# d-f/nylon-amt

Measured on AMD Instinct MI355X. Metric: training clips/sec (128-frame x 256-bin), higher is better.
Workload: dtype f16x3 (split fp16 / bf16 operand pairs, three bf16-rate MFMA passes per product, fp32 accumulate; tensors that flow between kernels are fp32 (attention q/k/v as fp16 hi+lo pairs), the copies SAVED only for the backward -- FFN hidden, its gradient, pre-LayerNorm sums -- are bf16); 1 GPU; paper-size hFT-Transformer training step (d=256, ff=512, 3+3 layers, 4 heads), batch 8 clips/GPU, dropout 0.10, forward+loss+backward+Adam; global_batch=8, frames=128, bins=256, parallelism=dp1, precision_mode=x3

## Files before the change

### nylon-amt_amd/csrc/x3_strip.hip

```cpp
#include <stdlib.h>
#include <type_traits>
#include <utility>
#include "hftt_common.h"
#include "x3_common.h"
#include "hftt_launch.h"
#include "x3_internal.h"
#include "../../include/hftt_hip.h"

#ifdef HFTT_X3_STRIP_ABLATE
#define XDBG(g, bit) (((g).pad & (bit)) != 0)
#else
#define XDBG(g, bit) false
#endif

namespace {

#include "strip_pipe.h"

__host__ __device__ inline int x3_i_of_c(int c) { const int g = c & 15, hh = c >> 4; return (g & 3) + 8 * (g >> 2) + 4 * hh; }

template <int E>
__global__ __launch_bounds__(256) void x3_strip_pack_kernel(const float* __restrict__ params, unsigned short* __restrict__ dst,
                                                            const hftt_strip_pack_entry* __restrict__ table) {
  const hftt_strip_pack_entry e = table[blockIdx.y];
  const int nrows = e.transpose ? e.cols : e.rows;
  const int nk = e.transpose ? e.rows : e.cols;
  const int kch = nk >> 3;
  const long total = (long)nrows * kch;
  for (long t = (long)blockIdx.x * 256 + threadIdx.x; t < total; t += (long)gridDim.x * 256) {
    const int nl = (int)(t / kch), kc = (int)(t - (long)nl * kch);
    const int n = e.n0 + nl, k = e.k0 + kc * 8;
    float v[8];
    const float* src = params + e.src_off;
    if (e.transpose) {
#pragma unroll
      for (int q = 0; q < 8; q++) v[q] = src[(long)(kc * 8 + q) * e.src_ld + nl];
    } else {
      const float4 a = *reinterpret_cast<const float4*>(src + (long)nl * e.src_ld + kc * 8);
      const float4 b = *reinterpret_cast<const float4*>(src + (long)nl * e.src_ld + kc * 8 + 4);
      v[0] = a.x; v[1] = a.y; v[2] = a.z; v[3] = a.w; v[4] = b.x; v[5] = b.y; v[6] = b.z; v[7] = b.w;
    }
    const int tile = n >> 5, i = x3_i_of_c(n & 31);
    const int pt = k >> 5, hk2 = (k >> 4) & 1, u = (k >> 3) & 1;
    const int ch = 2 * pt + u;
    long off;
    if (e.order == 2) {
      off = (e.slot_offset + (long)ch * e.slot_stride + tile) * 1024 + (hk2 * 32 + i) * 8;
    } else {
      long slot, frag;
      if (e.order == 0) { slot = (long)(tile >> 3) * (e.K >> 4) + ch; frag = 2 * (tile & 7); }
      else { slot = 2 * tile + (ch >> 3); frag = 2 * (ch & 7); }
      const long pos = e.slot_offset + (long)e.slot_stride * (slot >> 1) + (slot & 1);
      off = (pos * 16 + frag) * 512 + (hk2 * 32 + i) * 8;
    }
    bf16x8 hi, lo;
    x3_split8_checked<E>(v, hi, lo);
    *reinterpret_cast<bf16x8*>(dst + e.dst_off + off) = hi;
    *reinterpret_cast<bf16x8*>(dst + e.dst_off + off + 512) = lo;
  }
}

struct XPipe {
  const unsigned short* w;
  int S;
  int fill_pos;
  unsigned ring;
  int wave, lane;
  bool nofill, nobar;
  __device__ __forceinline__ const unsigned short* src_of(int pos) const { return w + ((long)pos * 16 + wave * 4) * 512 + lane * 8; }
  __device__ __forceinline__ void advance() { fill_pos = (fill_pos + 1 == S) ? 0 : fill_pos + 1; }
  template <int BUF>
  __device__ __forceinline__ void fill() {
    glds16x4(src_of(fill_pos), ring + (unsigned)BUF * SLOT_BYTES + (unsigned)wave * 4096u);
    advance();
  }
  __device__ __forceinline__ void begin_slot() {
    if (!nobar) { HFTT_WAITVM(4); __builtin_amdgcn_s_barrier(); }
  }
  __device__ __forceinline__ void prologue_sync() { HFTT_WAITVM(4); __builtin_amdgcn_s_barrier(); }
  template <int BUF>
  __device__ __forceinline__ void refill() {
    if (!nofill) glds16x4(src_of(fill_pos), ring + (unsigned)((BUF + FILL_AHEAD) & (NSLOT - 1)) * SLOT_BYTES + (unsigned)wave * 4096u);
    advance();
  }
  __device__ __forceinline__ void drain() { HFTT_WAITVM(0); }
};

struct XChunk { u4v a, b; };
#ifndef HFTT_STRIP_NT
#define HFTT_STRIP_NT 2
#endif
__device__ __forceinline__ u4v stream_load16(const void* p) {
#if HFTT_STRIP_NT == 1
  return __builtin_nontemporal_load(reinterpret_cast<const u4v*>(p));
#else
  return *reinterpret_cast<const u4v*>(p);
#endif
}
__device__ __forceinline__ void stream_store16(void* p, const u4v& v) {
#if HFTT_STRIP_NT
  __builtin_nontemporal_store(v, reinterpret_cast<u4v*>(p));
#else
  *reinterpret_cast<u4v*>(p) = v;
#endif
}
__device__ __forceinline__ void chunk_load(XChunk& c, const float* p) {
  c.a = stream_load16(p);
  c.b = stream_load16(p + 4);
}
template <typename V>
__device__ __forceinline__ void chunk_raw(XChunk& c, const V& v, int at = 0) {
  c.a = u4v{__float_as_uint(v[at]), __float_as_uint(v[at + 1]), __float_as_uint(v[at + 2]), __float_as_uint(v[at + 3])};
  c.b = u4v{__float_as_uint(v[at + 4]), __float_as_uint(v[at + 5]), __float_as_uint(v[at + 6]), __float_as_uint(v[at + 7])};
}
__device__ __forceinline__ void chunk_floats(const XChunk& c, float* v) {
  v[0] = __uint_as_float(c.a.x); v[1] = __uint_as_float(c.a.y); v[2] = __uint_as_float(c.a.z); v[3] = __uint_as_float(c.a.w);
  v[4] = __uint_as_float(c.b.x); v[5] = __uint_as_float(c.b.y); v[6] = __uint_as_float(c.b.z); v[7] = __uint_as_float(c.b.w);
}
template <int E>
__device__ __forceinline__ void x3_split16(const float* v, XChunk (&hf)[2]) {
#pragma unroll
  for (int u = 0; u < 2; u++) {
    bf16x8 hi, lo;
    x3_split8<E>(v + 8 * u, hi, lo);
    hf[u].a = __builtin_bit_cast(u4v, hi); hf[u].b = __builtin_bit_cast(u4v, lo);
  }
}
template <int E>
__device__ __forceinline__ void chunk_convert(XChunk& c) {
  float v[8];
  chunk_floats(c, v);
  bf16x8 hi, lo;
  if (E == X3_BF16H) {
    uint4 h;
    h.x = X3<E>::pk(v[0], v[1]); h.y = X3<E>::pk(v[2], v[3]); h.z = X3<E>::pk(v[4], v[5]); h.w = X3<E>::pk(v[6], v[7]);
    c.a = __builtin_bit_cast(u4v, h);
    return;
  }
  x3_split8<E>(v, hi, lo);
  c.a = __builtin_bit_cast(u4v, hi); c.b = __builtin_bit_cast(u4v, lo);
}
__device__ __forceinline__ void chunk_drop(XChunk& c, uint64_t seed, uint32_t site, uint64_t q0, uint32_t thr, float inv_keep) {
  float v[8];
  chunk_floats(c, v);
  drop8(v, seed, site, q0, thr, inv_keep);
  chunk_raw(c, v);
}
template <int E>
__device__ __forceinline__ void chunk_values(const XChunk& c, float* v) {
  const unsigned h[4] = {c.a.x, c.a.y, c.a.z, c.a.w}, l[4] = {c.b.x, c.b.y, c.b.z, c.b.w};
#pragma unroll
  for (int q = 0; q < 4; q++) {
    float h0, h1, l0, l1;
    X3<E>::unpk(h[q], h0, h1); X3<E>::unpk(l[q], l0, l1);
    v[2 * q] = h0 + l0; v[2 * q + 1] = h1 + l1;
  }
}
__device__ __forceinline__ int chunk_off(int ch) { return (ch >> 1) * 32 + (ch & 1) * 8; }

struct XPre { bf16x8 f[4]; bool noread = false; };
__device__ __forceinline__ void slot_head(const unsigned char* slot, XPre& pre) {
#pragma unroll
  for (int i = 0; i < 4; i++) pre.f[i] = *reinterpret_cast<const bf16x8*>(slot + i * 1024);
}
template <int E, typename G>
__device__ __forceinline__ void x3_slot_tiles(const unsigned char* slot, const unsigned char* next, XPre& pre, const XChunk& x, f32x16 (&acc)[8], G&& side) {
  bf16x8 fr[16];
#pragma unroll
  for (int i = 0; i < 4; i++) fr[i] = pre.f[i];
  const bf16x8 xh = __builtin_bit_cast(bf16x8, x.a), xl = __builtin_bit_cast(bf16x8, x.b);
  static_for<8>([&](auto t_c) __attribute__((always_inline)) {
    constexpr int t = decltype(t_c)::value;
    acc[t] = X3<E>::mma(fr[2 * t + 1], xh, acc[t]);
    side(std::integral_constant<int, 3 * t>{});
    if (pre.noread) { if (2 * t + 4 < 16) fr[2 * t + 4] = fr[2 * t]; }
    else if (2 * t + 4 < 16) fr[2 * t + 4] = *reinterpret_cast<const bf16x8*>(slot + (2 * t + 4) * 1024);
    else pre.f[2 * t + 4 - 16] = *reinterpret_cast<const bf16x8*>(next + (2 * t + 4 - 16) * 1024);
    if (E != X3_BF16H) acc[t] = X3<E>::mma(fr[2 * t], xl, acc[t]);
    side(std::integral_constant<int, 3 * t + 1>{});
    if (pre.noread) { if (2 * t + 5 < 16) fr[2 * t + 5] = fr[2 * t + 1]; }
    else if (2 * t + 5 < 16) fr[2 * t + 5] = *reinterpret_cast<const bf16x8*>(slot + (2 * t + 5) * 1024);
    else pre.f[2 * t + 5 - 16] = *reinterpret_cast<const bf16x8*>(next + (2 * t + 5 - 16) * 1024);
    acc[t] = X3<E>::mma(fr[2 * t], xh, acc[t]);
    side(std::integral_constant<int, 3 * t + 2>{});
    __builtin_amdgcn_sched_barrier(0);
  });
}
template <int E, int OFF, typename G>
__device__ __forceinline__ void x3_slot_chunks(const unsigned char* slot, const unsigned char* next, XPre& pre, const XChunk (&x)[16], f32x16& acc, G&& side) {
  bf16x8 fr[16];
#pragma unroll
  for (int i = 0; i < 4; i++) fr[i] = pre.f[i];
  static_for<8>([&](auto q_c) __attribute__((always_inline)) {
    constexpr int q = decltype(q_c)::value;
    const bf16x8 xh = __builtin_bit_cast(bf16x8, x[OFF + q].a), xl = __builtin_bit_cast(bf16x8, x[OFF + q].b);
    acc = X3<E>::mma(fr[2 * q + 1], xh, acc);
    side(std::integral_constant<int, 3 * q>{});
    if (pre.noread) { if (2 * q + 4 < 16) fr[2 * q + 4] = fr[2 * q]; }
    else if (2 * q + 4 < 16) fr[2 * q + 4] = *reinterpret_cast<const bf16x8*>(slot + (2 * q + 4) * 1024);
    else pre.f[2 * q + 4 - 16] = *reinterpret_cast<const bf16x8*>(next + (2 * q + 4 - 16) * 1024);
    if (E != X3_BF16H) acc = X3<E>::mma(fr[2 * q], xl, acc);
    side(std::integral_constant<int, 3 * q + 1>{});
    if (pre.noread) { if (2 * q + 5 < 16) fr[2 * q + 5] = fr[2 * q + 1]; }
    else if (2 * q + 5 < 16) fr[2 * q + 5] = *reinterpret_cast<const bf16x8*>(slot + (2 * q + 5) * 1024);
    else pre.f[2 * q + 5 - 16] = *reinterpret_cast<const bf16x8*>(next + (2 * q + 5 - 16) * 1024);
    acc = X3<E>::mma(fr[2 * q], xh, acc);
    side(std::integral_constant<int, 3 * q + 2>{});
    __builtin_amdgcn_sched_barrier(0);
  });
}

__device__ __forceinline__ f32x16 acc_from_lds(const float* row) {
  float b[16];
  lds16f(row, b);
  f32x16 acc;
#pragma unroll
  for (int q = 0; q < 16; q++) acc[q] = b[q];
  return acc;
}
__device__ __forceinline__ void acc_from_lds(f32x16 (&acc)[8], const float* row) {
#pragma unroll
  for (int ot = 0; ot < 8; ot++) acc[ot] = acc_from_lds(row + ot * 32);
}

__device__ __forceinline__ void load16f(const float* p, float* v) {
#pragma unroll
  for (int q = 0; q < 4; q++) { const float4 t = reinterpret_cast<const float4*>(p)[q]; v[4 * q] = t.x; v[4 * q + 1] = t.y; v[4 * q + 2] = t.z; v[4 * q + 3] = t.w; }
}
__device__ __forceinline__ void store16f(float* p, const float* v) {
#pragma unroll
// ... 231 lines not shown
          tile_store_rows(stage, v, j, hb, lane, cwave + ot * 32, g.ldc, wave_ok && !dbg_nostore);
        }
        __builtin_amdgcn_sched_barrier(0);
      }
      if (LN) {
        const bool p16 = g.flags & HFTT_SL_PRE_BF16;
        x3_ln_rows(acc, prm_b + g.N, prm_b + g.N + 256, hb, g.ln_mean, g.ln_rstd, tok, wave_ok, stage, j, lane,
                   (preb != nullptr && !p16) ? preb + (blk * 128 + wave * 32) * g.ldc : nullptr, cwave, g.ldc,
                   (preb != nullptr && p16) ? reinterpret_cast<unsigned short*>(preb) + (blk * 128 + wave * 32) * g.ldc : nullptr);
      }
    }
  }
  P.drain();
}

template <int E, int NT, bool HR, bool PLN = false, bool XD = false>
__global__ __launch_bounds__(256, 2) void x3_linear_n_kernel(const hftt_strip_desc g) {
  static_assert(!PLN || (E == X3_F16 && !HR), "f16-pair output: a forward projection without residual");
  static_assert(!XD || (E != X3_F16 && !PLN), "masked strip: a backward product");
  extern __shared__ __attribute__((aligned(16))) unsigned char smem[];
  const int tid = threadIdx.x, lane = tid & 63;
  const int wave = __builtin_amdgcn_readfirstlane(tid >> 6);
  const int j = lane & 31, h = lane >> 5;
  const long nblk = ((long)g.M + 127) / 128;
  float* prm = reinterpret_cast<float*>(smem + RING_BYTES);
  float* stage = reinterpret_cast<float*>(smem + RING_BYTES + 4 * NT * 32 + wave * STG_BYTES_PER_WAVE);
  const float* xb = reinterpret_cast<const float*>(g.x);
  float* cb = reinterpret_cast<float*>(g.C);
  const float* rb = reinterpret_cast<const float*>(g.residual);
  const bool relu = g.flags & HFTT_SL_RELU;
  const bool dbg_nostore = XDBG(g, 16);

  auto tok_of = [&](long blk) { const long t = blk * 128 + wave * 32 + j; return t < g.M ? t : (long)g.M - 1; };
  for (int i = tid; i < g.N; i += 256) prm[i] = g.bias != nullptr ? g.bias[i] : 0.f;
  XChunk xr[16];
  XPipe P = x3_open(g.w, 2 * NT, smem, wave, lane, XDBG(g, 1), XDBG(g, 2), xr, xb + tok_of(blockIdx.x) * g.ldx + 16 * h);

  const uint32_t thr = hftt_keep_thr(g.drop_p);
  const float inv_keep = hftt_keep_scale(g.drop_p);
  const unsigned char* abase = smem + lane * 16;
  for (long blk = blockIdx.x; blk < nblk; blk += gridDim.x) {
    int hb = h;
    asm volatile("" : "+v"(hb));
    const bool wave_ok = (blk * 128 + wave * 32) < g.M;
    const long nxt = blk + gridDim.x;
    auto lane_tok = [&](long b) { int l_ = lane; asm volatile("" : "+v"(l_)); const long t = b * 128 + wave * 32 + (l_ & 31); return t < g.M ? t : (long)g.M - 1; };
    float* cwave = cb + (blk * 128 + wave * 32) * g.ldc;
    int zero = 0;
    asm volatile("" : "+s"(zero));
    const float* prm_b = prm + zero;
    if (XD && g.drop_p > 0.f) {
      const uint64_t rowq_x = ((uint64_t)lane_tok(blk) * (uint64_t)g.K) >> 2;
#pragma unroll
      for (int c = 0; c < 16; c++) chunk_drop(xr[c], g.drop_seed, g.drop_site, rowq_x + ((chunk_off(c) + 16 * hb) >> 2), thr, inv_keep);
    }
#pragma unroll
    for (int c = 0; c < 16; c++) chunk_convert<E>(xr[c]);
    XPre pre;
    slot_head(abase, pre);

    for (int tp = 0; tp < NT / 2; tp++)
    static_for<2>([&](auto hf_c) __attribute__((always_inline)) {
      constexpr int half = decltype(hf_c)::value;
      constexpr int BA = (2 * half) & 3, BB = (2 * half + 1) & 3;
      const int t = 2 * tp + half;
      const bool LAST = (t == NT - 1);
      f32x16 hacc;
      {
        float b[16];
        lds16f(prm_b + t * 32 + 16 * hb, b);
#pragma unroll
        for (int q = 0; q < 16; q++) hacc[q] = b[q];
      }
      float r[16];
      P.begin_slot();
      x3_slot_chunks<E, 0>(abase + BA * SLOT_BYTES, abase + BB * SLOT_BYTES, pre, xr, hacc, [&](auto i_c) __attribute__((always_inline)) {
        constexpr int i = decltype(i_c)::value;
        if (i == 1) P.template refill<BA>();
        if (i == 4 && HR) {
          const long tokc = lane_tok(blk);
          const long rrow = g.res_mod > 0 ? (long)((unsigned)tokc % (unsigned)g.res_mod) : tokc;
          load16f(rb + rrow * g.ldr + 16 * hb + t * 32, r);
        }
        if (LAST && i % 3 == 2) chunk_load(xr[i / 3], xb + lane_tok(nxt < nblk ? nxt : blk) * g.ldx + 16 * hb + chunk_off(i / 3));
      });
      P.begin_slot();
      x3_slot_chunks<E, 8>(abase + BB * SLOT_BYTES, abase + ((BB + 1) & 3) * SLOT_BYTES, pre, xr, hacc, [&](auto i_c) __attribute__((always_inline)) {
        constexpr int i = decltype(i_c)::value;
        if (i == 1) P.template refill<BB>();
        if (LAST && i % 3 == 2) chunk_load(xr[8 + i / 3], xb + lane_tok(nxt < nblk ? nxt : blk) * g.ldx + 16 * hb + chunk_off(8 + i / 3));
      });
      float v[16];
#pragma unroll
      for (int q = 0; q < 16; q++) {
        float a = hacc[q];
        if (relu) a = fmaxf(a, 0.f);
        v[q] = a * g.out_scale;
      }
      if (!XD && g.drop_p > 0.f) {
        int l_ = lane; asm volatile("" : "+v"(l_));
        const uint64_t rowq = ((uint64_t)(blk * 128 + wave * 32 + (l_ & 31)) * (uint64_t)g.N) >> 2;
        drop16(v, g.drop_seed, g.drop_site, rowq + ((t * 32 + 16 * hb) >> 2), thr, inv_keep);
      }
      if (HR) {
#pragma unroll
        for (int q = 0; q < 16; q++) v[q] += r[q];
      }
      if (PLN) tile_store_rows_f16pair(stage, v, j, hb, lane, cwave + t * 32, g.ldc, wave_ok && !dbg_nostore);
      else tile_store_rows(stage, v, j, hb, lane, cwave + t * 32, g.ldc, wave_ok && !dbg_nostore);
    });
  }
  P.drain();
}

struct XNoHead {};
template <int MODE, int PT, bool HH, bool GH, bool HEAD, typename O>
__device__ __forceinline__ void x3_mlp_block(const O& o, const hftt_ffn_desc& g) {
  static_assert(!HEAD || MODE == 0, "the fc_o head belongs to the forward block");
  constexpr int E = (MODE == 0) ? X3_F16 : (GH ? X3_BF16H : X3_BF16);
  extern __shared__ __attribute__((aligned(16))) unsigned char smem[];
  const int tid = threadIdx.x, lane = tid & 63;
  const int wave = __builtin_amdgcn_readfirstlane(tid >> 6);
  const int j = lane & 31, h = lane >> 5;
  constexpr int p = PT * 32;
  constexpr int HP = HEAD ? 768 : 0;
  const long nblk = ((long)g.M + 127) / 128;
  float* prm_head = reinterpret_cast<float*>(smem + RING_BYTES);
  float* prm = prm_head + HP;
  float* stage = reinterpret_cast<float*>(smem + RING_BYTES + 4 * (HP + PT * 32 + 768) + wave * STG_BYTES_PER_WAVE);
  const float* xb;
  long ldx;
  if constexpr (HEAD) { xb = reinterpret_cast<const float*>(o.x); ldx = o.ldx; }
  else { xb = reinterpret_cast<const float*>(g.x); ldx = g.ldx; }
  float* yb = reinterpret_cast<float*>(g.y);
  float* preb = reinterpret_cast<float*>(g.pre_ln_out);
  const float* rb = reinterpret_cast<const float*>(g.residual);
  float* hob = reinterpret_cast<float*>(g.h_out);
  const float* gtb = reinterpret_cast<const float*>(g.gate);
  unsigned short* hob16 = reinterpret_cast<unsigned short*>(g.h_out);
  const unsigned short* gtb16 = reinterpret_cast<const unsigned short*>(g.gate);
  const bool has_res = (MODE == 1) && g.residual != nullptr;

  auto tok_of = [&](long blk) { const long t = blk * 128 + wave * 32 + j; return t < g.M ? t : (long)g.M - 1; };

  if constexpr (HEAD) {
    prm_head[tid] = o.bias != nullptr ? o.bias[tid] : 0.f;
    prm_head[256 + tid] = o.ln_gamma[tid]; prm_head[512 + tid] = o.ln_beta[tid];
  }
  for (int i = tid; i < p; i += 256) prm[i] = (MODE == 0 && g.b1 != nullptr) ? g.b1[i] : 0.f;
  prm[p + tid] = (MODE == 0 && g.b2 != nullptr) ? g.b2[tid] : 0.f;
  if (MODE == 0) { prm[p + 256 + tid] = g.ln_gamma[tid]; prm[p + 512 + tid] = g.ln_beta[tid]; }

  XChunk xr[16];
  const unsigned short* wstream;
  if constexpr (HEAD) wstream = o.w; else wstream = g.w;
  XPipe P = x3_open(wstream, (HEAD ? 16 : 0) + 4 * PT, smem, wave, lane, XDBG(g, 1), XDBG(g, 2), xr, xb + tok_of(blockIdx.x) * ldx + 16 * h);

  const uint32_t thr = hftt_keep_thr(g.drop_p);
  const float inv_keep = hftt_keep_scale(g.drop_p);
  uint32_t thr_a = 0;
  float inv_keep_a = 1.f;
  if constexpr (HEAD) { thr_a = hftt_keep_thr(o.drop_p); inv_keep_a = hftt_keep_scale(o.drop_p); }
  const unsigned char* abase = smem + lane * 16;
  for (long blk = blockIdx.x; blk < nblk; blk += gridDim.x) {
    int hb = h;
    asm volatile("" : "+v"(hb));
    const long tok = blk * 128 + wave * 32 + j;
    const bool wave_ok = (blk * 128 + wave * 32) < g.M;
    const long tokc = tok_of(blk);
    const long nxt = blk + gridDim.x;
    int zero = 0;
    asm volatile("" : "+s"(zero));
    const float* prm_b = prm + zero;
    const float* xrow_next = xb + (nxt < nblk ? tok_of(nxt) : tokc) * ldx + 16 * hb;
    const uint64_t rowq_h = ((uint64_t)tok * (uint64_t)p) >> 2;

    if constexpr (HEAD) {
      const float* prm_a = prm_b - HP;
      chunk_convert<E>(xr[0]);
      f32x16 acc[8];
      acc_from_lds(acc, prm_a + 16 * hb);
      XPre pre;
      slot_head(abase, pre);
      x3_kouter_slots<E>(P, abase, pre, xr, acc, false, true, nullptr, nullptr);
      const uint64_t rowq_a = ((uint64_t)tok * 256ull) >> 2;
      const long rrow = o.res_mod > 0 ? (long)((unsigned)tokc % (unsigned)o.res_mod) : tokc;
      const float* rrow_p = reinterpret_cast<const float*>(o.residual) + rrow * o.ldr + 16 * hb;
      float rnext[16];
      load16f(rrow_p, rnext);
#pragma unroll
      for (int ot = 0; ot < 8; ot++) {
        const int col0 = ot * 32 + 16 * hb;
        float v[16], r[16];
#pragma unroll
        for (int q = 0; q < 16; q++) r[q] = rnext[q];
        if (ot < 7) load16f(rrow_p + (ot + 1) * 32, rnext);
#pragma unroll
        for (int q = 0; q < 16; q++) v[q] = acc[ot][q] * o.out_scale;
        if (o.drop_p > 0.f) drop16(v, o.drop_seed, o.drop_site, rowq_a + (col0 >> 2), thr_a, inv_keep_a);
#pragma unroll
        for (int q = 0; q < 16; q++) acc[ot][q] = v[q] + r[q];
        __builtin_amdgcn_sched_barrier(0);
      }
      float* pre1b = reinterpret_cast<float*>(o.pre_ln_out);
      float* y1b = reinterpret_cast<float*>(o.C);
      const bool p16a = o.flags & HFTT_SL_PRE_BF16;
      x3_ln_rows<true>(acc, prm_a + 256, prm_a + 512, hb, o.ln_mean, o.ln_rstd, tok, wave_ok, stage, j, lane,
                       (pre1b != nullptr && !p16a) ? pre1b + (blk * 128 + wave * 32) * o.ldc : nullptr,
                       y1b != nullptr ? y1b + (blk * 128 + wave * 32) * o.ldc : nullptr, o.ldc,
                       (pre1b != nullptr && p16a) ? reinterpret_cast<unsigned short*>(pre1b) + (blk * 128 + wave * 32) * o.ldc : nullptr);
#pragma unroll
      for (int c = 0; c < 16; c++) { chunk_raw(xr[c], acc[c >> 1], 8 * (c & 1)); chunk_convert<E>(xr[c]); }
    } else {
      if (MODE == 1 && g.drop_p > 0.f) {
        const uint64_t rowq_x = ((uint64_t)tokc * 256ull) >> 2;
#pragma unroll
        for (int c = 0; c < 16; c++) chunk_drop(xr[c], g.drop_seed, g.site_o, rowq_x + ((chunk_off(c) + 16 * hb) >> 2), thr, inv_keep);
      }
#pragma unroll
      for (int c = 0; c < 16; c++) chunk_convert<E>(xr[c]);
    }

    f32x16 yacc[8];
    acc_from_lds(yacc, prm_b + p + 16 * hb);
    float gnext[16];
    if (MODE == 1) { if (HH) load16h(gtb16 + tokc * g.ldg + 16 * hb, gnext); else load16f(gtb + tokc * g.ldg + 16 * hb, gnext); }

    XPre pre;
    pre.noread = XDBG(g, 2048);
    slot_head(abase, pre);
    for (int t = 0; t < PT; t++) {
      f32x16 hacc;
      hacc = acc_from_lds(prm_b + t * 32 + 16 * hb);
      float gcur[16];
      if (MODE == 1) {
#pragma unroll
        for (int q = 0; q < 16; q++) gcur[q] = gnext[q];
      }
      P.begin_slot();
      if (!XDBG(g, 256))
      x3_slot_chunks<E, 0>(abase + 0 * SLOT_BYTES, abase + 1 * SLOT_BYTES, pre, xr, hacc, [&](auto i_c) __attribute__((always_inline)) {
        constexpr int i = decltype(i_c)::value;
        if (i == 1) P.template refill<0>();
        if (i == 6 && MODE == 1 && t + 1 < PT) {
          if (HH) load16h(gtb16 + tokc * g.ldg + (t + 1) * 32 + 16 * hb, gnext); else load16f(gtb + tokc * g.ldg + (t + 1) * 32 + 16 * hb, gnext);
        }
      });
      P.begin_slot();
      if (!XDBG(g, 256))
      x3_slot_chunks<E, 8>(abase + 1 * SLOT_BYTES, abase + 2 * SLOT_BYTES, pre, xr, hacc, [&](auto i_c) __attribute__((always_inline)) {
        constexpr int i = decltype(i_c)::value;
        if (i == 1) P.template refill<1>();
      });
      float v[16];
      const int hcol0 = t * 32 + 16 * hb;
      if (MODE == 0) {
#pragma unroll
        for (int q = 0; q < 16; q++) v[q] = fmaxf(hacc[q], 0.f);
        if (g.drop_p > 0.f && !XDBG(g, 128)) drop16(v, g.drop_seed, g.site_h, rowq_h + (hcol0 >> 2), thr, inv_keep);
      } else {
#pragma unroll
        for (int q = 0; q < 16; q++) v[q] = gcur[q] > 0.f ? hacc[q] * g.gate_scale : 0.f;
      }
      XChunk hf[2];
      if (XDBG(g, 1024)) {
        chunk_raw(hf[0], hacc, 0); chunk_raw(hf[1], hacc, 8);
      } else {
        x3_split16<E>(v, hf);
      }
      const bool st_h = hob != nullptr;
      float* hwave = hob + (blk * 128 + wave * 32) * g.ldh + t * 32;
      unsigned short* hwave16 = hob16 + (blk * 128 + wave * 32) * g.ldh + t * 32;
      P.begin_slot();
      if (!XDBG(g, 512))
      x3_slot_tiles<E>(abase + 2 * SLOT_BYTES, abase + 3 * SLOT_BYTES, pre, hf[0], yacc, [&](auto i_c) __attribute__((always_inline)) {
        constexpr int i = decltype(i_c)::value;
        if (i == 1) P.template refill<2>();
        if (i == 4 && st_h) {
          if (HH) tile_store_rows_bf16(stage, v, j, hb, lane, hwave16, g.ldh, wave_ok && !XDBG(g, 16));
          else tile_store_rows(stage, v, j, hb, lane, hwave, g.ldh, wave_ok && !XDBG(g, 16));
        }
      });
      P.begin_slot();
      if (!XDBG(g, 512))
      x3_slot_tiles<E>(abase + 3 * SLOT_BYTES, abase + 0 * SLOT_BYTES, pre, hf[1], yacc, [&](auto i_c) __attribute__((always_inline)) {
        constexpr int i = decltype(i_c)::value;
        if (i == 1) P.template refill<3>();
      });
    }

    const uint64_t rowq = ((uint64_t)tok * 256ull) >> 2;
    float* ywave = yb + (blk * 128 + wave * 32) * g.ldy;
    const float* rrow_p = rb + (has_res ? tokc * g.ldr + 16 * hb : 0);
#pragma unroll
    for (int ot = 0; ot < 8; ot++) {
      const int col0 = ot * 32 + 16 * hb;
      float v[16];
#pragma unroll
      for (int q = 0; q < 16; q++) v[q] = yacc[ot][q];
      if (MODE == 0 && g.drop_p > 0.f) drop16(v, g.drop_seed, g.site_o, rowq + (col0 >> 2), thr, inv_keep);
      if (MODE == 0) {
        float r[16];
        chunk_values<E>(xr[2 * ot], r); chunk_values<E>(xr[2 * ot + 1], r + 8);
#pragma unroll
        for (int q = 0; q < 16; q++) v[q] += r[q];
      } else if (has_res) {
        float r[16];
        load16f(rrow_p + ot * 32, r);
#pragma unroll
        for (int q = 0; q < 16; q++) v[q] += r[q];
      }
      chunk_load(xr[2 * ot], xrow_next + chunk_off(2 * ot));
      chunk_load(xr[2 * ot + 1], xrow_next + chunk_off(2 * ot + 1));
      if (MODE == 0) {
#pragma unroll
        for (int q = 0; q < 16; q++) yacc[ot][q] = v[q];
      } else {
        tile_store_rows(stage, v, j, hb, lane, ywave + ot * 32, g.ldy, wave_ok);
      }
      __builtin_amdgcn_sched_barrier(0);
    }
    if (MODE == 0) {
      const bool p16 = g.flags & HFTT_SL_PRE_BF16;
      x3_ln_rows(yacc, prm_b + p + 256, prm_b + p + 512, hb, g.ln_mean, g.ln_rstd, tok, wave_ok, stage, j, lane,
                 (preb != nullptr && !p16) ? preb + (blk * 128 + wave * 32) * g.ldy : nullptr, ywave, g.ldy,
                 (preb != nullptr && p16) ? reinterpret_cast<unsigned short*>(preb) + (blk * 128 + wave * 32) * g.ldy : nullptr);
    }
  }
  P.drain();
}
template <int MODE, int PT, bool HH, bool GH>
__global__ __launch_bounds__(256, 1) void x3_mlp_kernel(const hftt_ffn_desc g) { x3_mlp_block<MODE, PT, HH, GH, false>(XNoHead{}, g); }
template <bool HH>
__global__ __launch_bounds__(256, 1) void x3_oln_mlp_kernel(const hftt_strip_desc o, const hftt_ffn_desc g) { x3_mlp_block<0, 16, HH, false, true>(o, g); }

#ifndef HFTT_XL_XR
#define HFTT_XL_XR 8
#endif
template <int E, bool LN, int PASSES, int KCH, bool HR>
int launch_xl(const hftt_strip_desc& d, hipStream_t st) {
  constexpr int XR = (PASSES == 1 && !LN) ? HFTT_XL_XR : 16;
  const int lds = RING_BYTES + 4 * (PASSES * 256 + 512) + 4 * STG_BYTES_PER_WAVE;
  const long grid = hftt_persistent_grid("x3_strip_linear", ((long)d.M + 127) / 128, XR == 16 ? 1 : 2);
  if (grid < 0) return 2;
  return hftt_launch<x3_linear_kernel<E, LN, PASSES, KCH, HR, XR>>("x3_strip_linear", dim3((unsigned)grid), dim3(256), lds, st, d);
}
template <int E, int NT, bool HR, bool PLN = false, bool XD = false>
int launch_xn(const hftt_strip_desc& d, hipStream_t st) {
  const int lds = RING_BYTES + 4 * d.N + 4 * STG_BYTES_PER_WAVE;
  const long grid = hftt_persistent_grid("x3_strip_linear", ((long)d.M + 127) / 128, 2);
  if (grid < 0) return 2;
  return hftt_launch<x3_linear_n_kernel<E, NT, HR, PLN, XD>>("x3_strip_linear", dim3((unsigned)grid), dim3(256), lds, st, d);
}
template <int MODE, bool HH, bool GH = false>
int launch_xm(const hftt_ffn_desc& d, hipStream_t st) {
  const int lds = RING_BYTES + 4 * (d.p + 768) + 4 * STG_BYTES_PER_WAVE;
  const long grid = hftt_persistent_grid("x3_strip_mlp", ((long)d.M + 127) / 128, 1);
  if (grid < 0) return 2;
  return hftt_launch<x3_mlp_kernel<MODE, 16, HH, GH>>("x3_strip_mlp", dim3((unsigned)grid), dim3(256), lds, st, d);
}

template <bool HH>
int launch_xom(const hftt_strip_desc& o, const hftt_ffn_desc& d, hipStream_t st) {
  const int lds = RING_BYTES + 4 * 2048 + 4 * STG_BYTES_PER_WAVE;
  const long grid = hftt_persistent_grid("x3_attn_out_ffn", ((long)d.M + 127) / 128, 1);
  if (grid < 0) return 2;
  return hftt_launch<x3_oln_mlp_kernel<HH>>("x3_attn_out_ffn", dim3((unsigned)grid), dim3(256), lds, st, o, d);
}

template <int E>
struct X3Stream {
  using Chunk = XChunk;
  static constexpr int PAIR_BYTES = 2048;
  static constexpr int STAGE_BYTES = STG_BYTES_PER_WAVE;
  static constexpr const char* LINEAR_WHAT = "x3s_strip_linear";
  static constexpr const char* MLP_WHAT = "x3s_strip_mlp";
  static constexpr bool STAGES_OUTSIDE = true;
  static constexpr int wgs(int lds_bytes) { return lds_bytes <= 52 * 1024 ? 3 : (lds_bytes <= 78 * 1024 ? 2 : 1); }

  static __device__ __forceinline__ void copy_weights(unsigned char* lds, const unsigned short* w, int pairs, int tid) {
    const uint4* src = reinterpret_cast<const uint4*>(w);
    uint4* dst = reinterpret_cast<uint4*>(lds);
    for (int i = tid; i < pairs * 128; i += 256) dst[i] = src[i];
  }
  template <int KC>
  static __device__ __forceinline__ void load_strip(XChunk (&xr)[KC], const void* x, long off) {
    const float* p0 = reinterpret_cast<const float*>(x) + off;
#pragma unroll
    for (int c = 0; c < KC; c++) chunk_load(xr[c], p0 + chunk_off(c));
#pragma unroll
    for (int c = 0; c < KC; c++) chunk_convert<E>(xr[c]);
  }
  static __device__ __forceinline__ void tile_mac(const unsigned char* wl, int pair, const XChunk& x, f32x16& acc) {
    const unsigned char* p = wl + pair * 2048;
    const bf16x8 fh = *reinterpret_cast<const bf16x8*>(p), fl = *reinterpret_cast<const bf16x8*>(p + 1024);
    const bf16x8 xh = __builtin_bit_cast(bf16x8, x.a), xl = __builtin_bit_cast(bf16x8, x.b);
    acc = X3<E>::mma(fl, xh, acc);
    acc = X3<E>::mma(fh, xl, acc);
    acc = X3<E>::mma(fh, xh, acc);
  }
  static __device__ __forceinline__ void load16(const void* base, long off, bool h16, float* v) {
    if (h16) load16h(reinterpret_cast<const unsigned short*>(base) + off, v);
    else load16f(reinterpret_cast<const float*>(base) + off, v);
  }
  static __device__ __forceinline__ void values8(const XChunk& c, float* v) { chunk_values<E>(c, v); }
  static __device__ __forceinline__ void split16(const float* v, XChunk (&hf)[2]) { x3_split16<E>(v, hf); }
  static __device__ __forceinline__ void* rows(void* base, long off, bool h16) {
    return h16 ? static_cast<void*>(reinterpret_cast<unsigned short*>(base) + off) : static_cast<void*>(reinterpret_cast<float*>(base) + off);
  }
  static __device__ __forceinline__ void emit(unsigned char* stg, const float* v, int j, int hb, int lane, void* rows, long ld, int t, bool ok, bool h16) {
    float* stage = reinterpret_cast<float*>(stg);
    if (h16) tile_store_rows_bf16(stage, v, j, hb, lane, reinterpret_cast<unsigned short*>(rows) + t * 32, ld, ok);
    else tile_store_rows(stage, v, j, hb, lane, reinterpret_cast<float*>(rows) + t * 32, ld, ok);
  }
  template <int K32, int NT, bool LN, bool HR>
  static int launch_linear(dim3 grid, int lds, hipStream_t st, const hftt_strip_desc& d);
  template <int MODE, bool HH>
  static int launch_mlp(dim3 grid, int lds, hipStream_t st, const hftt_ffn_desc& d);
};

#include "small_strip.h"

template <int E, int K32, int NT, bool LN, bool HR>
__global__ __launch_bounds__(256, X3Stream<E>::wgs(SmallCfg<X3Stream<E>, K32, NT, LN>::LDS)) void x3s_linear_kernel(const hftt_strip_desc g) {
  extern __shared__ __attribute__((aligned(16))) unsigned char smem[];
  small_linear<X3Stream<E>, K32, NT, LN, HR>(g, smem);
}
template <int MODE> using X3MlpStream = X3Stream<(MODE == 0) ? X3_F16 : X3_BF16>;
template <int MODE, bool HH>
__global__ __launch_bounds__(256, 2) void x3s_mlp_kernel(const hftt_ffn_desc g) {
  extern __shared__ __attribute__((aligned(16))) unsigned char smem[];
  small_mlp<X3MlpStream<MODE>, MODE, HH>(g, smem);
}
template <int E>
template <int K32, int NT, bool LN, bool HR>
int X3Stream<E>::launch_linear(dim3 grid, int lds, hipStream_t st, const hftt_strip_desc& d) {
  return hftt_launch<x3s_linear_kernel<E, K32, NT, LN, HR>>(LINEAR_WHAT, grid, dim3(256), lds, st, d);
}
template <int E>
template <int MODE, bool HH>
int X3Stream<E>::launch_mlp(dim3 grid, int lds, hipStream_t st, const hftt_ffn_desc& d) {
  return hftt_launch<x3s_mlp_kernel<MODE, HH>>(MLP_WHAT, grid, dim3(256), lds, st, d);
}

template <int E>
int dispatch_xl(const hftt_strip_desc& d, hipStream_t st) {
  const int passes = d.N / 256, kch = d.K / 256;
  const bool hr = d.residual != nullptr;
#define HFTT_XL(LN_, P_, K_) return hr ? launch_xl<E, LN_, P_, K_, true>(d, st) : launch_xl<E, LN_, P_, K_, false>(d, st)
  if (d.ln_gamma != nullptr) {
    if (kch == 1) HFTT_XL(true, 1, 1);
    if (kch == 2) HFTT_XL(true, 1, 2);
    hftt_set_error("x3_strip_linear: the LayerNorm form covers K = 256 / 512 (got %d)", d.K);
    return 1;
  }
  if constexpr (E == X3_F16) {
    if (d.flags & HFTT_SL_C_F16PAIR) {
      if (passes == 1) return launch_xn<E, 8, false, true>(d, st);
      if (passes == 2) return launch_xn<E, 16, false, true>(d, st);
      if (passes == 3) return launch_xn<E, 24, false, true>(d, st);
      if (passes == 4) return launch_xn<E, 32, false, true>(d, st);
      if (passes == 6) return launch_xn<E, 48, false, true>(d, st);
      hftt_set_error("x3_strip_linear: the plane form covers N = 256, 512, 768, 1024, 1536 (got %d)", d.N);
      return 1;
    }
  }
  if constexpr (E == X3_BF16) {
    if (d.flags & HFTT_SL_X_DROP) return launch_xn<E, 8, false, false, true>(d, st);
  }
  if (kch == 1 && passes == 1) return hr ? launch_xn<E, 8, true>(d, st) : launch_xn<E, 8, false>(d, st);
  if (kch == 1 && passes == 2) return hr ? launch_xn<E, 16, true>(d, st) : launch_xn<E, 16, false>(d, st);
  if (kch == 1 && passes == 3) return hr ? launch_xn<E, 24, true>(d, st) : launch_xn<E, 24, false>(d, st);
  if (kch == 2 && passes == 1) HFTT_XL(false, 1, 2);
  if (kch == 3 && passes == 1) HFTT_XL(false, 1, 3);
#undef HFTT_XL
  hftt_set_error("x3_strip_linear: shape N=%d K=%d is not covered (N/256 x K/256 in {1x1, 2x1, 3x1, 1x2, 1x3})", d.N, d.K);
  return 1;
}

}
// ... 109 lines not shown
```

Baseline: 301.2 clips/s.

## Prefetch gate and residual rows earlier in backward FFN strip kernel

```diff
diff --git a/nylon-amt_amd/csrc/x3_strip.hip b/nylon-amt_amd/csrc/x3_strip.hip
--- a/nylon-amt_amd/csrc/x3_strip.hip
+++ b/nylon-amt_amd/csrc/x3_strip.hip
@@ -76,6 +76,9 @@
   }
   __device__ __forceinline__ void begin_slot() {
     if (!nobar) { HFTT_WAITVM(4); __builtin_amdgcn_s_barrier(); }
+  }
+  __device__ __forceinline__ void begin_slot(bool behind32) {
+    if (!nobar) { if (behind32) HFTT_WAITVM(36); else HFTT_WAITVM(4); __builtin_amdgcn_s_barrier(); }
   }
   __device__ __forceinline__ void prologue_sync() { HFTT_WAITVM(4); __builtin_amdgcn_s_barrier(); }
   template <int BUF>
@@ -613,9 +616,16 @@
   if (MODE == 0) { prm[p + 256 + tid] = g.ln_gamma[tid]; prm[p + 512 + tid] = g.ln_beta[tid]; }
 
   XChunk xr[16];
+  u4v gnext[HH ? 2 : 4];
+  auto gate_load = [&](long row, int col) __attribute__((always_inline)) {
+    const void* gp = HH ? static_cast<const void*>(gtb16 + row * g.ldg + col) : static_cast<const void*>(gtb + row * g.ldg + col);
+#pragma unroll
+    for (int q = 0; q < (HH ? 2 : 4); q++) gnext[q] = reinterpret_cast<const u4v*>(gp)[q];
+  };
   const unsigned short* wstream;
   if constexpr (HEAD) wstream = o.w; else wstream = g.w;
   XPipe P = x3_open(wstream, (HEAD ? 16 : 0) + 4 * PT, smem, wave, lane, XDBG(g, 1), XDBG(g, 2), xr, xb + tok_of(blockIdx.x) * ldx + 16 * h);
+  if (MODE == 1) gate_load(tok_of(blockIdx.x), 16 * h);
 
   const uint32_t thr = hftt_keep_thr(g.drop_p);
   const float inv_keep = hftt_keep_scale(g.drop_p);
@@ -635,6 +645,7 @@
     const float* prm_b = prm + zero;
     const float* xrow_next = xb + (nxt < nblk ? tok_of(nxt) : tokc) * ldx + 16 * hb;
     const uint64_t rowq_h = ((uint64_t)tok * (uint64_t)p) >> 2;
+    const float* rrow_p = rb + (has_res ? tokc * g.ldr + 16 * hb : 0);
 
     if constexpr (HEAD) {
       const float* prm_a = prm_b - HP;
@@ -684,8 +695,6 @@
 
     f32x16 yacc[8];
     acc_from_lds(yacc, prm_b + p + 16 * hb);
-    float gnext[16];
-    if (MODE == 1) { if (HH) load16h(gtb16 + tokc * g.ldg + 16 * hb, gnext); else load16f(gtb + tokc * g.ldg + 16 * hb, gnext); }
 
     XPre pre;
     pre.noread = XDBG(g, 2048);
@@ -693,19 +702,11 @@
     for (int t = 0; t < PT; t++) {
       f32x16 hacc;
       hacc = acc_from_lds(prm_b + t * 32 + 16 * hb);
-      float gcur[16];
-      if (MODE == 1) {
-#pragma unroll
-        for (int q = 0; q < 16; q++) gcur[q] = gnext[q];
-      }
       P.begin_slot();
       if (!XDBG(g, 256))
       x3_slot_chunks<E, 0>(abase + 0 * SLOT_BYTES, abase + 1 * SLOT_BYTES, pre, xr, hacc, [&](auto i_c) __attribute__((always_inline)) {
         constexpr int i = decltype(i_c)::value;
         if (i == 1) P.template refill<0>();
-        if (i == 6 && MODE == 1 && t + 1 < PT) {
-          if (HH) load16h(gtb16 + tokc * g.ldg + (t + 1) * 32 + 16 * hb, gnext); else load16f(gtb + tokc * g.ldg + (t + 1) * 32 + 16 * hb, gnext);
-        }
       });
       P.begin_slot();
       if (!XDBG(g, 256))
@@ -720,6 +721,12 @@
         for (int q = 0; q < 16; q++) v[q] = fmaxf(hacc[q], 0.f);
         if (g.drop_p > 0.f && !XDBG(g, 128)) drop16(v, g.drop_seed, g.site_h, rowq_h + (hcol0 >> 2), thr, inv_keep);
       } else {
+        float gcur[16];
+        if (HH) { unpack8(gnext[0], gcur); unpack8(gnext[1], gcur + 8); }
+        else {
+#pragma unroll
+          for (int q = 0; q < 16; q++) gcur[q] = __uint_as_float(gnext[q >> 2][q & 3]);
+        }
 #pragma unroll
         for (int q = 0; q < 16; q++) v[q] = gcur[q] > 0.f ? hacc[q] * g.gate_scale : 0.f;
       }
@@ -729,10 +736,16 @@
       } else {
         x3_split16<E>(v, hf);
       }
+      const bool res_issued = has_res && t == PT - 1;
+      if (MODE == 1) asm volatile("" : "+v"(hf[0].a), "+v"(hf[0].b), "+v"(hf[1].a), "+v"(hf[1].b)::"memory");
+      if (res_issued) {
+#pragma unroll
+        for (int c = 0; c < 16; c++) chunk_load(xr[c], rrow_p + chunk_off(c));
+      }
       const bool st_h = hob != nullptr;
       float* hwave = hob + (blk * 128 + wave * 32) * g.ldh + t * 32;
       unsigned short* hwave16 = hob16 + (blk * 128 + wave * 32) * g.ldh + t * 32;
-      P.begin_slot();
+      P.begin_slot(res_issued);
       if (!XDBG(g, 512))
       x3_slot_tiles<E>(abase + 2 * SLOT_BYTES, abase + 3 * SLOT_BYTES, pre, hf[0], yacc, [&](auto i_c) __attribute__((always_inline)) {
         constexpr int i = decltype(i_c)::value;
@@ -741,8 +754,9 @@
           if (HH) tile_store_rows_bf16(stage, v, j, hb, lane, hwave16, g.ldh, wave_ok && !XDBG(g, 16));
           else tile_store_rows(stage, v, j, hb, lane, hwave, g.ldh, wave_ok && !XDBG(g, 16));
         }
+        if (i == 6 && MODE == 1 && t + 1 < PT) gate_load(tokc, (t + 1) * 32 + 16 * hb);
       });
-      P.begin_slot();
+      P.begin_slot(res_issued);
       if (!XDBG(g, 512))
       x3_slot_tiles<E>(abase + 3 * SLOT_BYTES, abase + 0 * SLOT_BYTES, pre, hf[1], yacc, [&](auto i_c) __attribute__((always_inline)) {
         constexpr int i = decltype(i_c)::value;
@@ -752,7 +766,6 @@
 
     const uint64_t rowq = ((uint64_t)tok * 256ull) >> 2;
     float* ywave = yb + (blk * 128 + wave * 32) * g.ldy;
-    const float* rrow_p = rb + (has_res ? tokc * g.ldr + 16 * hb : 0);
 #pragma unroll
     for (int ot = 0; ot < 8; ot++) {
       const int col0 = ot * 32 + 16 * hb;
@@ -767,7 +780,7 @@
         for (int q = 0; q < 16; q++) v[q] += r[q];
       } else if (has_res) {
         float r[16];
-        load16f(rrow_p + ot * 32, r);
+        chunk_floats(xr[2 * ot], r); chunk_floats(xr[2 * ot + 1], r + 8);
 #pragma unroll
         for (int q = 0; q < 16; q++) v[q] += r[q];
       }
@@ -781,12 +794,17 @@
       }
       __builtin_amdgcn_sched_barrier(0);
     }
+    if (MODE == 1) gate_load(nxt < nblk ? tok_of(nxt) : tokc, 16 * hb);
     if (MODE == 0) {
       const bool p16 = g.flags & HFTT_SL_PRE_BF16;
       x3_ln_rows(yacc, prm_b + p + 256, prm_b + p + 512, hb, g.ln_mean, g.ln_rstd, tok, wave_ok, stage, j, lane,
                  (preb != nullptr && !p16) ? preb + (blk * 128 + wave * 32) * g.ldy : nullptr, ywave, g.ldy,
                  (preb != nullptr && p16) ? reinterpret_cast<unsigned short*>(preb) + (blk * 128 + wave * 32) * g.ldy : nullptr);
     }
+  }
+  if (MODE == 1) {
+    if (HH) asm volatile("" ::"v"(gnext[0]), "v"(gnext[1]));
+    else asm volatile("" ::"v"(gnext[0]), "v"(gnext[1]), "v"(gnext[2]), "v"(gnext[3]));
   }
   P.drain();
 }
```

Result: no change. 302.2 clips/s, median of 6 (+0.3%).
